# sehyun03/MulActSeg

Measured on AMD Instinct MI355X. Metric: superpixels scored/sec, higher is better.
Workload: dtype f32; 1 GPU; acquisition-round: PixBal+ban-ignore scorer on resident logits, Cityscapes pool shape [4,20,1024,2048] per step; per rank K single-pass scans (class prior + region sums + histograms) of its shard, then exchange 1 (all-gather class sums) + device class weights (k_class_weight) + weighted finalize + ban + exchange 2 (all-gather scores) + replicated K4 (keys, radix sort, fair-counting budget walk) ov; nseg=2048, id_dtype=int64, regions_scored=679936, budget_clicks=11159, regions_selected=6688

## Files before the change

include/mulactseg_hip.h:

```cpp
#ifndef MULACTSEG_HIP_H
#define MULACTSEG_HIP_H

#include <stddef.h>
#include <stdint.h>

#ifdef __cplusplus
extern "C" {
#endif

#define MAS_ID_I64 0
#define MAS_ID_I32 1
#define MAS_ID_U16 2
#define MAS_MAP_U8 3

#define MAS_MAX_CLASSES 32

#define MAS_SCORE_FRAC_BITS 40
#define MAS_PROB_FRAC_BITS 23
#define MAS_LOSS_FRAC_BITS 32

#define MAS_ABI_VERSION 9
int mas_abi_version(void);
const char* mas_error_string(int code);

// ... 54 lines not shown
#define MAS_GRAD_FRAC_BITS 44
int mas_fix_to_float(const int64_t* fix, int64_t n, int frac_bits, float* out, void* stream);

size_t mas_partial_loss_work_bytes(int N, int S, int C, int flags);
int mas_partial_loss_fwd_fused(const float* z, int h, int w, const void* spx, int spx_dtype, const uint8_t* mask, const uint8_t* targets,
                               int cols_stored, int cols_used, const uint32_t* bits, int N, int C, int H, int W, int S, float invT, int flags,
                               const float* weights, void* work, size_t work_bytes, float* losses, void* stream);
int mas_partial_loss_bwd_fused(const float* z, int h, int w, const void* spx, int spx_dtype, const uint8_t* mask, const uint32_t* bits,
                               const void* work, const float* grad, const float* weights, int N, int C, int H, int W, int S, float invT,
                               int flags, float* dz, int64_t* dzq_fix, void* stream);


int mas_region_keys(const float* score, const uint8_t* valid, const int32_t* img_rank, int64_t n_img, int S,
                    uint64_t* keys , void* stream);

size_t mas_select_workspace_bytes(int64_t n);

int mas_sort_keys_desc(const uint64_t* keys_in, int64_t n, uint64_t* keys_out, void* workspace, size_t ws_bytes,
                       void* stream);

int mas_budget_walk(const uint64_t* sorted_keys, int64_t n, const uint8_t* region_cost, const int32_t* img_of_rank,
                    int S, int64_t budget, int64_t max_out, int64_t* n_selected,
                    int32_t* sel_img, int32_t* sel_id, float* sel_score, void* workspace, size_t ws_bytes, void* stream);

int mas_region_reweight(float* score, const int32_t* dominant, int64_t n, int ban_class, const float* cls_w ,
                        void* stream);

int mas_dominant_hist(const int32_t* dominant, int64_t n, int C, uint64_t* counts , void* stream);

int mas_minmax_normalize(float* scores, int64_t n, uint32_t* scratch2, void* stream);


#define MAS_LABELS_BAD_VALUE 1

int mas_region_label_counts(const void* spx, int spx_dtype, const uint8_t* labels, int H, int W, int nseg, int num_classes, int trim_k,
                            int32_t* full , int32_t* trimmed , int32_t* status ,
                            void* stream);

int mas_region_multi_hot(const int32_t* full, const int32_t* trimmed, const uint8_t* listed, int nseg, int num_classes,
                         uint8_t* bits , int64_t* size , void* stream);

int mas_region_dominant(const int32_t* full, const uint8_t* listed, const int32_t* drawn , int nseg, int num_classes,
                        int generate_ignore, int32_t* choice , void* stream);

int mas_region_paint(const void* spx, int spx_dtype, const uint8_t* labels, int H, int W, int nseg, const int32_t* choice,
                     int generate_ignore, uint8_t* out , void* stream);
// ... 202 lines not shown
```

mulactseg_amd/_lib.py:

```python
import ctypes
import os

_HERE = os.path.dirname(os.path.abspath(__file__))
LIB_PATH = os.environ.get("MAS_LIB") or os.path.join(_HERE, "libmulactseg_hip.so")

ID_I64, ID_I32, ID_U16 = 0, 1, 2
MAP_U8 = 3
MAX_CLASSES = 32
LABELS_BAD_VALUE = 1
SCORE_FRAC, PROB_FRAC, LOSS_FRAC = 40, 23, 32
LOSS_CE, LOSS_GROUP, LOSS_GROUP_ONLY_MULTI, LOSS_DECOMP, LOSS_TCE = 1, 2, 4, 8, 16
ACC_WORDS = 8
GRAD_FRAC = 44
MS_MAX_SOURCES = 16

SK_DMA, SK_NOSPLIT = 1, 2
LOWRES_GENERIC = 1
STAGE2_THR_MEDIAN, STAGE2_THR_MIN = 0, 1
ABI_VERSION = 9

_c = ctypes
_vp, _i, _f, _i64, _d = _c.c_void_p, _c.c_int, _c.c_float, _c.c_int64, _c.c_double


class SkOpts(ctypes.Structure):
    _fields_ = [("flags", _c.c_uint), ("spin_limit", _c.c_uint), ("stamps", _c.c_void_p)]


SIGNATURES = {
    "mas_abi_version": (_i, []),
    "mas_error_string": (_c.c_char_p, [_i]),
    "mas_class_prob_sum": (_i, [_vp, _i, _i, _i, _i, _f, _vp, _vp]),
    "mas_bvsb_region_accum": (_i, [_vp, _vp, _i, _vp, _i, _i, _i, _i, _i, _f, _vp, _vp, _vp]),
    "mas_region_finalize": (_i, [_vp, _vp, _i64, _i, _i, _vp, _vp, _vp, _vp, _vp]),
    "mas_region_keys": (_i, [_vp, _vp, _vp, _i64, _i, _vp, _vp]),
    "mas_select_workspace_bytes": (_c.c_size_t, [_i64]),
    "mas_sort_keys_desc": (_i, [_vp, _i64, _vp, _vp, _c.c_size_t, _vp]),
    "mas_budget_walk": (_i, [_vp, _i64, _vp, _vp, _i, _i64, _i64, _vp, _vp, _vp, _vp, _vp, _c.c_size_t, _vp]),
    "mas_region_reweight": (_i, [_vp, _vp, _i64, _i, _vp, _vp]),
    "mas_dominant_hist": (_i, [_vp, _i64, _i, _vp, _vp]),
    "mas_minmax_normalize": (_i, [_vp, _i64, _vp, _vp]),
    "mas_region_label_counts": (_i, [_vp, _i, _vp, _i, _i, _i, _i, _i, _vp, _vp, _vp, _vp]),
    "mas_region_multi_hot": (_i, [_vp, _vp, _vp, _i, _i, _vp, _vp, _vp]),
    "mas_region_dominant": (_i, [_vp, _vp, _vp, _i, _i, _i, _vp, _vp]),
    "mas_region_paint": (_i, [_vp, _i, _vp, _i, _i, _i, _vp, _i, _vp, _vp]),
    "mas_spx_max_onehot": (_i, [_vp, _i, _vp, _i, _i, _i, _i, _i, _vp, _vp, _vp, _vp, _vp]),
    "mas_iou_counts": (_i, [_vp, _vp, _vp, _i64, _i, _i64, _vp, _vp]),
    "mas_logits_iou_counts": (_i, [_vp, _vp, _i, _i, _i, _i, _i, _i64, _vp, _vp]),
    "mas_lowres_iou_counts": (_i, [_vp, _vp, _i, _i, _i, _i, _i, _i, _i, _i64, _vp, _vp]),
    "mas_single_pass_accum": (_i, [_vp, _vp, _i, _i, _i, _i, _i, _i, _f, _vp, _vp, _vp, _vp]),
    "mas_single_pass_accum_lowres": (_i, [_vp, _i, _i, _vp, _i, _i, _i, _i, _i, _i, _f, _vp, _vp, _vp, _vp]),
    "mas_single_pass_accum_lowres_opt": (_i, [_vp, _i, _i, _vp, _i, _i, _i, _i, _i, _i, _f, _vp, _vp, _vp, _c.c_uint, _vp]),
    "mas_class_weight": (_i, [_vp, _i, _i, _i64, _i, _i, _d, _vp, _vp, _vp, _vp]),
    "mas_region_finalize_weighted": (_i, [_vp, _vp, _i64, _i, _vp, _i, _vp, _vp, _vp, _vp, _vp]),
    "mas_stage2_gather_protos": (_i, [_vp, _i, _i, _i, _i, _i, _vp, _i, _vp, _vp]),
    "mas_stage2_assign": (_i, [_vp, _i, _i, _i, _i, _i, _vp, _vp, _i, _vp, _vp, _vp, _vp, _vp]),
    "mas_stage2_adjacency": (_i, [_vp, _i, _i, _i, _vp, _vp, _vp]),
    "mas_stage2_propagate": (_i, [_vp, _i, _i, _i, _i, _i, _vp, _i, _vp, _vp, _vp, _vp, _vp, _vp, _vp, _vp]),
    "mas_stage2_thresholds_scratch_bytes": (_i64, [_i, _i]),
    "mas_stage2_thresholds": (_i, [_vp, _vp, _i, _i, _i, _vp, _i64, _vp, _vp]),
    "mas_aspp_dw3_fwd": (_i, [_vp, _vp, _vp, _vp, _i, _i, _i, _i, _i, _i, _i, _vp, _vp, _vp, _vp]),
# ... 135 lines not shown
```

mulactseg_amd/active_selection/engine.py:

```python
import numpy as np
import torch


class ShardPlan:

    def __init__(self, n_img, batch_size, rank=0, world=1):
        self.n_img, self.batch_size, self.rank, self.world = n_img, batch_size, rank, world
        self.n_batches = (n_img + batch_size - 1) // batch_size
        per = (self.n_batches + world - 1) // world
        self.batch_lo = min(rank * per, self.n_batches)
        self.batch_hi = min((rank + 1) * per, self.n_batches)
        self.img_lo = min(self.batch_lo * batch_size, n_img)
        self.img_hi = min(self.batch_hi * batch_size, n_img)
        self.per_rank_imgs = per * batch_size
        self.batch_of = (np.arange(n_img) // batch_size).astype(np.int32)

    @property
    def local_indices(self):
        return list(range(self.img_lo, self.img_hi))

    @property
    def n_local(self):
        return self.img_hi - self.img_lo

# ... 67 lines not shown

    def class_weight(self, prob_sum, hw, batch_size, n_batches, coeff):
        cum, w, w31 = self.ops.class_weight(prob_sum.contiguous(), hw, batch_size, n_batches, coeff)
        w._mas_w31 = w31
        return cum, w

    def finalize_weighted(self, class_sum, hist, cls_w, ban_class, want_hist_i64=False):
        w31 = None if cls_w is None else getattr(cls_w, '_mas_w31', None)
        if w31 is None:
            w = torch.ones(hist.shape[-1], dtype=torch.float32, device=hist.device) if cls_w is None else cls_w.detach().to(hist.device)
            w31 = (w.double() * 2147483648.0).floor().to(torch.int64).view(torch.int32)[::2].contiguous()
        return self.ops.region_finalize_weighted(class_sum, hist, w31, ban_class, want_hist_i64)

    def minmax_normalize_(self, scores):
        return self.ops.minmax_normalize_(scores)

    def region_reweight_(self, scores, dominant, ban_class, cls_w):
        return self.ops.region_reweight_(scores, dominant, ban_class, cls_w)

    def dominant_hist(self, dominant, C):
        return self.ops.dominant_hist(dominant, C)

    def select(self, scores, valid, img_rank, img_of_rank, region_cost, budget, max_out):
        keys = self.ops.region_keys(scores, valid, img_rank)
        skeys = self.ops.sort_keys_desc(keys)
        nsel, simg, sid, ssc = self.ops.budget_walk(skeys, region_cost, img_of_rank, scores.shape[1], budget, max_out)
        n = int(nsel.item())
        return n, simg[:n].cpu().numpy(), sid[:n].cpu().numpy(), ssc[:n].cpu().numpy()

    def local_head(self, plan, scores, valid, img_rank, max_out):
        lo, hi = plan.img_lo, plan.img_hi
        head = torch.zeros(max_out, dtype=torch.int64, device=scores.device)
        if hi > lo:
            keys = self.ops.region_keys(scores[lo:hi].contiguous(), None if valid is None else valid[lo:hi].contiguous(),
                                        img_rank[lo:hi].contiguous())
            m = min(keys.numel(), max_out)
            head[:m] = self.ops.sort_keys_desc(keys)[:m]
        return head

    def walk_heads(self, heads, region_cost, img_of_rank, S, budget, max_out):
        nsel, simg, sid, ssc = self.ops.budget_walk(self.ops.sort_keys_desc(heads), region_cost, img_of_rank, S, budget, max_out)
        n = int(nsel.item())
        return n, simg[:n].cpu().numpy(), sid[:n].cpu().numpy(), ssc[:n].cpu().numpy()

    def select_sharded(self, plan, scores, valid, img_rank, img_of_rank, region_cost, budget, max_out):
        head = self.local_head(plan, scores, valid, img_rank, max_out)
        merged = torch.empty(plan.world * max_out, dtype=torch.int64, device=scores.device)
        _dist().all_gather_into_tensor(merged, head)
        return self.walk_heads(merged, region_cost, img_of_rank, scores.shape[1], budget, max_out)


def default_backend(device):
    return HipBackend(device)


def select_regions(backend, plan, scores, valid, img_rank, img_of_rank, region_cost, budget, max_out):
    if plan.world > 1 and max_out is not None and _dist() is not None and hasattr(backend, 'select_sharded'):
        return backend.select_sharded(plan, scores, valid, img_rank, img_of_rank, region_cost, budget, max_out)
    return backend.select(scores, valid, img_rank, img_of_rank, region_cost, budget, max_out)


class AcquisitionRound:

    def __init__(self, n_img, n_channels, n_superpixels, batch_size, temperature, backend, rank=None, world=None,
                 single_pass=False):
        r, w = current_rank_world()
# ... 97 lines not shown
```

mulactseg_amd/csrc/select.hip:

```cpp
#include <cstring>

#include <rocprim/device/device_radix_sort.hpp>
#include <rocprim/device/device_scan.hpp>

#include "common.h"

namespace {

constexpr int kThreads = 256;

__device__ __forceinline__ unsigned order_bits(float f) {
    const unsigned b = mas_f2u(f);
    return (b & 0x80000000u) ? ~b : (b | 0x80000000u);
}
__device__ __forceinline__ float unorder_bits(unsigned o) {
    return mas_u2f((o & 0x80000000u) ? (o & 0x7fffffffu) : ~o);
}

inline int id_bits_for(int S) {
    int b = 1;
    while ((1LL << b) < S) ++b;
    return b;
}

// ... 100 lines not shown
        if (v != 0.0f) lo = o < lo ? o : lo;
        hi = o > hi ? o : hi;
    }
#pragma unroll
    for (int off = MAS_WAVE / 2; off > 0; off >>= 1) {
        const unsigned l2 = __shfl_down(lo, off, MAS_WAVE), h2 = __shfl_down(hi, off, MAS_WAVE);
        lo = l2 < lo ? l2 : lo;
        hi = h2 > hi ? h2 : hi;
    }
    if ((threadIdx.x & (MAS_WAVE - 1)) == 0) {
        atomicMin(&mm[0], lo);
        atomicMax(&mm[1], hi);
    }
}

__global__ void k_minmax_init(unsigned* mm) { mm[0] = 0xffffffffu; mm[1] = 0u; }

__global__ __launch_bounds__(kThreads) void k_minmax_apply(float* __restrict__ u, long long n, const unsigned* __restrict__ mm) {
    const long long i = (long long)blockIdx.x * kThreads + threadIdx.x;
    if (i >= n) return;
    const float mn = unorder_bits(mm[0]);
    const float mx = unorder_bits(mm[1]) - mn;
    u[i] = (u[i] - mn) / mx;
}

inline size_t align_up(size_t v) { return (v + 255) & ~(size_t)255; }

size_t sort_temp_bytes(long long n) {
    size_t bytes = 0;
    mas_u64* nul = nullptr;
    (void)rocprim::radix_sort_keys_desc(nullptr, bytes, nul, nul, (size_t)n, 0, 64, (hipStream_t)0);
    return bytes;
}
size_t scan_temp_bytes(long long n) {
    size_t bytes = 0;
    unsigned* nul = nullptr;
    (void)rocprim::inclusive_scan(nullptr, bytes, nul, nul, (size_t)n, rocprim::plus<unsigned>(), (hipStream_t)0);
    return bytes;
}

}

extern "C" size_t mas_select_workspace_bytes(int64_t n) {
    if (n <= 0) return 0;
    const size_t t = sort_temp_bytes(n), u = scan_temp_bytes(n);
    return align_up(t > u ? t : u) + 2 * align_up(sizeof(unsigned) * (size_t)n) + 256;
// ... 35 lines not shown
    hipStream_t st = static_cast<hipStream_t>(stream);
    const int b = id_bits_for(S);
    unsigned char* ws = static_cast<unsigned char*>(workspace);
    size_t temp = scan_temp_bytes(n);
    const size_t t = sort_temp_bytes(n);
    const size_t temp_region = align_up(t > temp ? t : temp);
    unsigned* cost = reinterpret_cast<unsigned*>(ws + temp_region);
    unsigned* prefix = reinterpret_cast<unsigned*>(ws + temp_region + align_up(sizeof(unsigned) * (size_t)n));
    const mas_u64* keys = reinterpret_cast<const mas_u64*>(sorted_keys);
    unsigned long long* nsel = reinterpret_cast<unsigned long long*>(n_selected);
    const long long nblk = (n + kThreads - 1) / kThreads;
    hipLaunchKernelGGL(k_set_u64, dim3(1), dim3(1), 0, st, nsel, (unsigned long long)n);
    hipLaunchKernelGGL(k_walk_cost, dim3((unsigned)nblk), dim3(kThreads), 0, st, keys, (long long)n, region_cost, img_of_rank, S, b, cost);
    hipError_t e = rocprim::inclusive_scan(ws, temp, cost, prefix, (size_t)n, rocprim::plus<unsigned>(), st);
    if (e != hipSuccess) return (int)e;
    hipLaunchKernelGGL(k_walk_find, dim3((unsigned)nblk), dim3(kThreads), 0, st, keys, prefix, (long long)n,
                       (unsigned long long)budget, nsel);
    const long long oblk = (max_out + kThreads - 1) / kThreads;
    hipLaunchKernelGGL(k_walk_emit, dim3((unsigned)oblk), dim3(kThreads), 0, st, keys, nsel, (long long)max_out, img_of_rank, b,
                       sel_img, sel_id, sel_score);
    return mas_launch_status();
}

extern "C" int mas_minmax_normalize(float* scores, int64_t n, uint32_t* scratch2, void* stream) {
    if (!scores || !scratch2) return MAS_ERR_NULL;
    if (n <= 0) return MAS_ERR_SHAPE;
    hipStream_t st = static_cast<hipStream_t>(stream);
    long long nblk = (n + kThreads - 1) / kThreads;
    hipLaunchKernelGGL(k_minmax_init, dim3(1), dim3(1), 0, st, scratch2);
    hipLaunchKernelGGL(k_minmax_nonzero, dim3((unsigned)(nblk > 1024 ? 1024 : nblk)), dim3(kThreads), 0, st, scores, (long long)n, scratch2);
    hipLaunchKernelGGL(k_minmax_apply, dim3((unsigned)nblk), dim3(kThreads), 0, st, scores, (long long)n, scratch2);
    return mas_launch_status();
}

extern "C" int mas_region_reweight(float* score, const int32_t* dominant, int64_t n, int ban_class, const float* cls_w, void* stream) {
    if (!score || !dominant) return MAS_ERR_NULL;
    if (n <= 0) return MAS_ERR_SHAPE;
    const long long nblk = (n + kThreads - 1) / kThreads;
    hipLaunchKernelGGL(k_region_reweight, dim3((unsigned)nblk), dim3(kThreads), 0, static_cast<hipStream_t>(stream), score, dominant,
                       (long long)n, ban_class, cls_w);
    return mas_launch_status();
}

extern "C" int mas_dominant_hist(const int32_t* dominant, int64_t n, int C, uint64_t* counts, void* stream) {
    if (!dominant || !counts) return MAS_ERR_NULL;
    if (n <= 0) return MAS_ERR_SHAPE;
// ... 8 lines not shown
```

mulactseg_amd/csrc/single_pass.hip:

```cpp
#include <cstdlib>
#include "common.h"

namespace {

constexpr int kThreads = 256;
constexpr int kTileW = 256;
constexpr int kTileH = 16;
constexpr int kLogSlots = 7;
constexpr int kSlots = 1 << kLogSlots;

__device__ __forceinline__ int table_slot(int* keys, int id) {
    unsigned h = ((unsigned)id * 2654435769u) >> (32 - kLogSlots);
    for (int probe = 0; probe < kSlots; ++probe) {
        int k = __hip_atomic_load(&keys[h], __ATOMIC_RELAXED, __HIP_MEMORY_SCOPE_WORKGROUP);
        if (k == id) return (int)h;
        if (k == -1) {
            int old = atomicCAS(&keys[h], -1, id);
            if (old == -1 || old == id) return (int)h;
        }
        h = (h + 1) & (kSlots - 1);
    }
    return -1;
}

// ... 481 lines not shown
                                                                        int C, const unsigned* __restrict__ w31, int ban_class,
                                                                        float* __restrict__ score, int* __restrict__ dominant,
                                                                        unsigned* __restrict__ count,
                                                                        long long* __restrict__ hist_i64) {
    extern __shared__ __attribute__((aligned(16))) unsigned char smem[];
    const int CP = C | 1;
    mas_u64* s_sum = reinterpret_cast<mas_u64*>(smem);
    unsigned* s_hist = reinterpret_cast<unsigned*>(s_sum + (size_t)kThreads * CP);
    const long long r0 = (long long)blockIdx.x * kThreads;
    const long long rows = (n_regions - r0) < kThreads ? (n_regions - r0) : kThreads;
    const long long words = rows * C;
    for (long long i = threadIdx.x; i < words; i += kThreads) {
        const int row = (int)(i / C), col = (int)(i - (long long)row * C);
        const unsigned hv = hist[r0 * C + i];
        s_sum[row * CP + col] = class_sum[r0 * C + i];
        s_hist[row * CP + col] = hv;
        if (hist_i64) hist_i64[r0 * C + i] = (long long)hv;
    }
    __syncthreads();
    if ((long long)threadIdx.x >= rows) return;
    const long long r = r0 + threadIdx.x;
    const unsigned* h = s_hist + threadIdx.x * CP;
    const mas_u64* cs = s_sum + threadIdx.x * CP;
    unsigned long long n = 0;
    unsigned best = 0;
    int arg = 0;
    uint64_t hi = 0, lo = 0;
    for (int c = 0; c < C; ++c) {
        const unsigned v = h[c];
        n += v;
        if (v > best) { best = v; arg = c; }
        if (v) mas_mac_u64_u32((uint64_t)cs[c], w31[c], &hi, &lo);
    }
    float sc = 0.0f;
    if (n) sc = mas_fixed_mean(mas_shr31_u128(hi, lo), n, MAS_SCORE_FRAC);
    if (ban_class >= 0 && arg == ban_class) sc = 0.0f;
    score[r] = sc;
    if (dominant) dominant[r] = arg;
    if (count) count[r] = (unsigned)n;
}

inline bool mas_ring_enabled() {
    static const bool on = [] { const char* e = getenv("MAS_SINGLE_PASS_RING"); return !(e && e[0] == '0'); }();
    return on;
}

// ... 122 lines not shown
    if (flags & ~MAS_LOWRES_GENERIC) return MAS_ERR_RANGE;
    hipStream_t st = static_cast<hipStream_t>(stream);
    mas_u64* ps = reinterpret_cast<mas_u64*>(prob_sum);
    mas_u64* cs = reinterpret_cast<mas_u64*>(class_sum);
    switch (C) {
        case 19: return dispatch_low_ids<19, true>(zq, h, w, spx, spx_dtype, B, C, H, W, S, invT, ps, cs, hist, flags, st);
        case 20: return dispatch_low_ids<20, true>(zq, h, w, spx, spx_dtype, B, C, H, W, S, invT, ps, cs, hist, flags, st);
        case 21: return dispatch_low_ids<21, true>(zq, h, w, spx, spx_dtype, B, C, H, W, S, invT, ps, cs, hist, flags, st);
        default: return MAS_ERR_CLASSES;
    }
}

extern "C" int mas_single_pass_accum_lowres(const float* zq, int h, int w, const void* spx, int spx_dtype, int B, int C, int H, int W, int S,
                                            float invT, uint64_t* prob_sum, uint64_t* class_sum, uint32_t* hist, void* stream) {
    return mas_single_pass_accum_lowres_opt(zq, h, w, spx, spx_dtype, B, C, H, W, S, invT, prob_sum, class_sum, hist, 0u, stream);
}

extern "C" int mas_region_finalize_weighted(const uint64_t* class_sum, const uint32_t* hist, int64_t n_regions, int C,
                                            const uint32_t* w31, int ban_class, float* score, int32_t* dominant, uint32_t* count,
                                            int64_t* hist_i64, void* stream) {
    if (!class_sum || !hist || !w31 || !score) return MAS_ERR_NULL;
    if (n_regions <= 0) return MAS_ERR_SHAPE;
    if (C < 1 || C > MAS_MAX_CLASSES) return MAS_ERR_CLASSES;
    const long long nblk = (n_regions + kThreads - 1) / kThreads;
    if (nblk > 0x7fffffffLL) return MAS_ERR_SHAPE;
    const size_t smem = (sizeof(mas_u64) + sizeof(unsigned)) * (size_t)kThreads * (C | 1);
    hipLaunchKernelGGL(k_region_finalize_weighted, dim3((unsigned)nblk), dim3(kThreads), smem, static_cast<hipStream_t>(stream),
                       reinterpret_cast<const mas_u64*>(class_sum), hist, (long long)n_regions, C, w31, ban_class, score, dominant,
                       count, reinterpret_cast<long long*>(hist_i64));
    return mas_launch_status();
}
```

mulactseg_amd/ops.py:

```python
import ctypes
import os

import numpy as np
import torch

from . import _lib

_ID_CODES = {torch.int64: _lib.ID_I64, torch.int32: _lib.ID_I32, torch.uint16: _lib.ID_U16,
             torch.int16: _lib.ID_U16}


def inv_temperature(T):
    return float(np.float32(1.0) / np.float32(T))


def _stream(t):
    return torch.cuda.current_stream(t.device).cuda_stream


def _need(t, name, dtype=None):
    if not t.is_cuda:
        raise _lib.MulActSegHipError("%s must live on the GPU (no CPU path exists)" % name)
    if dtype is not None and t.dtype != dtype:
        raise TypeError("%s must be %s, got %s" % (name, dtype, t.dtype))
# ... 282 lines not shown


def budget_walk(sorted_keys, region_cost, img_of_rank, S, budget, max_out=None):
    _need(sorted_keys, "sorted_keys", torch.int64)
    _need(img_of_rank, "img_of_rank", torch.int32)
    cost_bits = region_cost
    if cost_bits is not None:
        _need(cost_bits, "region_cost", torch.uint8)
    n = sorted_keys.numel()
    max_out = n if max_out is None else min(n, max_out)
    dev = sorted_keys.device
    lib = _lib.load()
    ws = torch.empty(lib.mas_select_workspace_bytes(n), dtype=torch.uint8, device=dev)
    nsel = torch.empty(1, dtype=torch.int64, device=dev)
    sel_img = torch.empty(max_out, dtype=torch.int32, device=dev)
    sel_id = torch.empty(max_out, dtype=torch.int32, device=dev)
    sel_score = torch.empty(max_out, dtype=torch.float32, device=dev)
    with torch.cuda.device(dev):
        _lib.check(lib.mas_budget_walk(sorted_keys.data_ptr(), n, cost_bits.data_ptr() if cost_bits is not None else None,
                                       img_of_rank.data_ptr(), S, int(budget), max_out, nsel.data_ptr(), sel_img.data_ptr(),
                                       sel_id.data_ptr(), sel_score.data_ptr(), ws.data_ptr(), ws.numel(), _stream(sorted_keys)),
                   "mas_budget_walk")
    return nsel, sel_img, sel_id, sel_score


def minmax_normalize_(scores):
    _need(scores, "scores", torch.float32)
    scratch = torch.empty(2, dtype=torch.int32, device=scores.device)
    with torch.cuda.device(scores.device):
        _lib.check(_lib.load().mas_minmax_normalize(scores.data_ptr(), scores.numel(), scratch.data_ptr(), _stream(scores)),
                   "mas_minmax_normalize")
    return scores


def iou_counts(outputs, outputs_all, targets, num_classes, ignore_label, counts=None):
    _need(targets, "targets", torch.int64)
    if outputs is not None:
        _need(outputs, "outputs", torch.int64)
    if outputs_all is not None:
        _need(outputs_all, "outputs_all", torch.int64)
    if counts is None:
        counts = torch.zeros(3 * num_classes + 3, dtype=torch.int64, device=targets.device)
    with torch.cuda.device(targets.device):
        _lib.check(_lib.load().mas_iou_counts(outputs.data_ptr() if outputs is not None else None,
                                              outputs_all.data_ptr() if outputs_all is not None else None,
                                              targets.data_ptr(), targets.numel(), num_classes, int(ignore_label),
# ... 1930 lines not shown
```

Before: 56.30 million superpixels/s.

## Replace full radix sort selection with histogram-threshold top-prefix select and fused sort-walk

Adds a prefix selection path. Two histogram passes over the score key bits find a threshold, a compaction pass keeps only the candidates above it (up to 8192), and one block runs a bitonic sort and the budget walk in shared memory, writing a single packed record. The aim is to avoid building and radix-sorting keys for all regions when only a few thousand can be selected. The record is read back in one pinned copy, and the path falls back to the full sort when candidates overflow the cap. The finalize kernel also gains a tiled variant, which adds complexity and possible tie and edge-case risks.

```diff
diff --git a/include/mulactseg_hip.h b/include/mulactseg_hip.h
--- a/include/mulactseg_hip.h
+++ b/include/mulactseg_hip.h
@@ -100,6 +100,12 @@
 int mas_budget_walk(const uint64_t* sorted_keys, int64_t n, const uint8_t* region_cost, const int32_t* img_of_rank,
                     int S, int64_t budget, int64_t max_out, int64_t* n_selected,
                     int32_t* sel_img, int32_t* sel_id, float* sel_score, void* workspace, size_t ws_bytes, void* stream);
+
+int64_t mas_select_prefix_cap(void);
+size_t mas_select_prefix_workspace_bytes(void);
+int mas_select_prefix(const float* score, const uint8_t* valid, const int32_t* img_rank, const int32_t* img_of_rank,
+                      const uint8_t* region_cost, int64_t n_img, int S, int64_t budget, int64_t max_out, int32_t* record,
+                      void* workspace, size_t ws_bytes, void* stream);
 
 int mas_region_reweight(float* score, const int32_t* dominant, int64_t n, int ban_class, const float* cls_w ,
                         void* stream);
diff --git a/mulactseg_amd/_lib.py b/mulactseg_amd/_lib.py
--- a/mulactseg_amd/_lib.py
+++ b/mulactseg_amd/_lib.py
@@ -37,6 +37,9 @@
     "mas_select_workspace_bytes": (_c.c_size_t, [_i64]),
     "mas_sort_keys_desc": (_i, [_vp, _i64, _vp, _vp, _c.c_size_t, _vp]),
     "mas_budget_walk": (_i, [_vp, _i64, _vp, _vp, _i, _i64, _i64, _vp, _vp, _vp, _vp, _vp, _c.c_size_t, _vp]),
+    "mas_select_prefix_cap": (_i64, []),
+    "mas_select_prefix_workspace_bytes": (_c.c_size_t, []),
+    "mas_select_prefix": (_i, [_vp, _vp, _vp, _vp, _vp, _i64, _i, _i64, _i64, _vp, _vp, _c.c_size_t, _vp]),
     "mas_region_reweight": (_i, [_vp, _vp, _i64, _i, _vp, _vp]),
     "mas_dominant_hist": (_i, [_vp, _i64, _i, _vp, _vp]),
     "mas_minmax_normalize": (_i, [_vp, _i64, _vp, _vp]),
diff --git a/mulactseg_amd/active_selection/engine.py b/mulactseg_amd/active_selection/engine.py
--- a/mulactseg_amd/active_selection/engine.py
+++ b/mulactseg_amd/active_selection/engine.py
@@ -113,11 +113,7 @@
         return self.ops.dominant_hist(dominant, C)
 
     def select(self, scores, valid, img_rank, img_of_rank, region_cost, budget, max_out):
-        keys = self.ops.region_keys(scores, valid, img_rank)
-        skeys = self.ops.sort_keys_desc(keys)
-        nsel, simg, sid, ssc = self.ops.budget_walk(skeys, region_cost, img_of_rank, scores.shape[1], budget, max_out)
-        n = int(nsel.item())
-        return n, simg[:n].cpu().numpy(), sid[:n].cpu().numpy(), ssc[:n].cpu().numpy()
+        return self.ops.select(scores, valid, img_rank, img_of_rank, region_cost, budget, max_out)
 
     def local_head(self, plan, scores, valid, img_rank, max_out):
         lo, hi = plan.img_lo, plan.img_hi
@@ -130,9 +126,7 @@
         return head
 
     def walk_heads(self, heads, region_cost, img_of_rank, S, budget, max_out):
-        nsel, simg, sid, ssc = self.ops.budget_walk(self.ops.sort_keys_desc(heads), region_cost, img_of_rank, S, budget, max_out)
-        n = int(nsel.item())
-        return n, simg[:n].cpu().numpy(), sid[:n].cpu().numpy(), ssc[:n].cpu().numpy()
+        return self.ops.walk_heads(heads, region_cost, img_of_rank, S, budget, max_out)
 
     def select_sharded(self, plan, scores, valid, img_rank, img_of_rank, region_cost, budget, max_out):
         head = self.local_head(plan, scores, valid, img_rank, max_out)
diff --git a/mulactseg_amd/csrc/select.hip b/mulactseg_amd/csrc/select.hip
--- a/mulactseg_amd/csrc/select.hip
+++ b/mulactseg_amd/csrc/select.hip
@@ -146,6 +146,267 @@
     const float mn = unorder_bits(mm[0]);
     const float mx = unorder_bits(mm[1]) - mn;
     u[i] = (u[i] - mn) / mx;
+}
+
+constexpr int kSelCap = 8192;
+constexpr int kSelBins = 4096;
+constexpr unsigned kNoBin = 0xffffffffu;
+constexpr int kSortThreads = 1024;
+constexpr int kSortItems = kSelCap / kSortThreads;
+constexpr int kHistItems = kSelBins / kThreads;
+enum { kStT1 = 0, kStAbove1, kStNeed2, kStM, kStCount, kStWords = 8 };
+constexpr size_t kSelStateBytes = 256;
+constexpr size_t kSelHistBytes = sizeof(unsigned) * kSelBins;
+constexpr size_t kSelZeroBytes = kSelStateBytes + 2 * kSelHistBytes;
+constexpr size_t kSelWorkspaceBytes = kSelZeroBytes + sizeof(mas_u64) * kSelCap;
+constexpr int kSortSlots = kSelCap + kSelCap / 8;
+constexpr size_t kSortSmemBytes = sizeof(mas_u64) * kSortSlots + sizeof(unsigned) * 32;
+
+__device__ __forceinline__ mas_u64 region_key(const float* __restrict__ score, const unsigned char* __restrict__ valid,
+                                              const int* __restrict__ img_rank, unsigned i, unsigned S, int id_bits) {
+    if (valid && !valid[i]) return 0;
+    const unsigned img = i / S;
+    const unsigned id = i - img * S;
+    const unsigned lo = ((unsigned)img_rank[img] << id_bits) | id;
+    return ((mas_u64)order_bits(score[i]) << 32) | lo;
+}
+
+__device__ void find_threshold(const unsigned* __restrict__ hist, unsigned need_cap, unsigned* s_scan, unsigned* out) {
+    const int tid = threadIdx.x;
+    unsigned h[kHistItems];
+    unsigned sum = 0;
+#pragma unroll
+    for (int e = 0; e < kHistItems; e += 4) {
+        const uint4 v = *reinterpret_cast<const uint4*>(hist + tid * kHistItems + e);
+        h[e] = v.x; h[e + 1] = v.y; h[e + 2] = v.z; h[e + 3] = v.w;
+        sum += v.x + v.y + v.z + v.w;
+    }
+    s_scan[tid] = sum;
+    if (tid == 0) { out[0] = kNoBin; out[1] = 0; }
+    __syncthreads();
+    for (int off = 1; off < kThreads; off <<= 1) {
+        const unsigned v = (tid + off < kThreads) ? s_scan[tid + off] : 0u;
+        __syncthreads();
+        s_scan[tid] += v;
+        __syncthreads();
+    }
+    const unsigned total = s_scan[0], incl = s_scan[tid], excl = incl - sum;
+    const unsigned need = need_cap < total ? need_cap : total;
+    if (need > 0 && excl < need && need <= incl) {
+        unsigned run = excl, T = kNoBin, above = 0;
+#pragma unroll
+        for (int e = kHistItems - 1; e >= 0; --e) {
+            if (T == kNoBin && run + h[e] >= need) { T = (unsigned)(tid * kHistItems + e); above = run; }
+            run += h[e];
+        }
+        out[0] = T;
+        out[1] = above;
+    }
+    if (tid == 0) out[2] = total;
+    __syncthreads();
+}
+
+template <int LEVEL>
+__global__ __launch_bounds__(kThreads) void k_prefix_hist(const float* __restrict__ score, const unsigned char* __restrict__ valid,
+                                                           const int* __restrict__ img_rank, unsigned n, unsigned S, int id_bits,
+                                                           unsigned max_out, unsigned* __restrict__ state,
+                                                           unsigned* __restrict__ hist1, unsigned* __restrict__ hist2) {
+    __shared__ unsigned s_h[kSelBins];
+    __shared__ unsigned s_scan[kThreads];
+    __shared__ unsigned s_out[4];
+    for (int b = threadIdx.x; b < kSelBins; b += kThreads) s_h[b] = 0;
+    unsigned T1 = 0;
+    if (LEVEL == 2) {
+        find_threshold(hist1, max_out, s_scan, s_out);
+        T1 = s_out[0];
+        if (blockIdx.x == 0 && threadIdx.x == 0) {
+            const unsigned need1 = max_out < s_out[2] ? max_out : s_out[2];
+            state[kStT1] = T1;
+            state[kStAbove1] = s_out[1];
+            state[kStNeed2] = need1 - s_out[1];
+        }
+        if (T1 == kNoBin) return;
+    }
+    __syncthreads();
+    for (unsigned long long i = (unsigned long long)blockIdx.x * kThreads + threadIdx.x; i < n; i += (unsigned long long)gridDim.x * kThreads) {
+        const mas_u64 k = region_key(score, valid, img_rank, (unsigned)i, S, id_bits);
+        if (LEVEL == 1) {
+            if (k) atomicAdd(&s_h[(unsigned)(k >> 52)], 1u);
+        } else {
+            if (k && (unsigned)(k >> 52) == T1) atomicAdd(&s_h[(unsigned)(k >> 40) & (kSelBins - 1)], 1u);
+        }
+    }
+    __syncthreads();
+    unsigned* hist = LEVEL == 1 ? hist1 : hist2;
+    for (int b = threadIdx.x; b < kSelBins; b += kThreads)
+        if (s_h[b]) atomicAdd(&hist[b], s_h[b]);
+}
+
+constexpr int kCompactItems = 4;
+
+__global__ __launch_bounds__(kThreads) void k_prefix_compact(const float* __restrict__ score, const unsigned char* __restrict__ valid,
+                                                              const int* __restrict__ img_rank, unsigned n, unsigned S, int id_bits,
+                                                              unsigned* __restrict__ state, const unsigned* __restrict__ hist2,
+                                                              mas_u64* __restrict__ cand) {
+    __shared__ unsigned s_scan[kThreads];
+    __shared__ unsigned s_out[4];
+    __shared__ unsigned s_wave[kThreads / MAS_WAVE + 1];
+    const unsigned T1 = state[kStT1];
+    if (T1 == kNoBin) return;
+    find_threshold(hist2, state[kStNeed2], s_scan, s_out);
+    const unsigned T2 = s_out[0];
+    if (T2 == kNoBin) return;
+    const unsigned m = state[kStAbove1] + s_out[1] + hist2[T2];
+    if (blockIdx.x == 0 && threadIdx.x == 0) state[kStM] = m;
+    if (m > (unsigned)kSelCap) return;
+    const unsigned cut = (T1 << 12) | T2;
+    const unsigned tid = threadIdx.x, lane = tid & (MAS_WAVE - 1), wave = tid / MAS_WAVE;
+    const unsigned long long i0 = (unsigned long long)blockIdx.x * (kThreads * kCompactItems) + tid;
+    mas_u64 k[kCompactItems];
+    unsigned cnt = 0;
+#pragma unroll
+    for (int e = 0; e < kCompactItems; ++e) {
+        const unsigned long long i = i0 + (unsigned)e * kThreads;
+        mas_u64 key = 0;
+        if (i < n) key = region_key(score, valid, img_rank, (unsigned)i, S, id_bits);
+        if (key == 0 || (unsigned)(key >> 40) < cut) key = 0;
+        k[e] = key;
+        cnt += key != 0;
+    }
+    unsigned incl = cnt;
+#pragma unroll
+    for (int off = 1; off < MAS_WAVE; off <<= 1) {
+        const unsigned up = __shfl_up(incl, off, MAS_WAVE);
+        if ((int)lane >= off) incl += up;
+    }
+    if (lane == MAS_WAVE - 1) s_wave[wave] = incl;
+    __syncthreads();
+    if (tid == 0) {
+        unsigned total = 0;
+#pragma unroll
+        for (int w = 0; w < kThreads / MAS_WAVE; ++w) { const unsigned c = s_wave[w]; s_wave[w] = total; total += c; }
+        s_wave[kThreads / MAS_WAVE] = total ? atomicAdd(&state[kStCount], total) : 0u;
+    }
+    __syncthreads();
+    unsigned at = s_wave[kThreads / MAS_WAVE] + s_wave[wave] + incl - cnt;
+#pragma unroll
+    for (int e = 0; e < kCompactItems; ++e) {
+        if (k[e]) {
+            if (at < (unsigned)kSelCap) cand[at] = k[e];
+            ++at;
+        }
+    }
+}
+
+__device__ __forceinline__ unsigned sort_slot(unsigned i) { return i + (i >> 3); }
+
+template <int STEPS>
+__device__ __forceinline__ void bitonic_group(mas_u64* s_key, unsigned P, unsigned k, unsigned j, unsigned tid) {
+    constexpr unsigned G = 1u << STEPS;
+    const unsigned jl = j >> (STEPS - 1);
+    for (unsigned g = tid; g < (P >> STEPS); g += kSortThreads) {
+        const unsigned base = ((g & ~(jl - 1)) << STEPS) | (g & (jl - 1));
+        const bool desc = (base & k) == 0;
+        mas_u64 v[G];
+#pragma unroll
+        for (unsigned a = 0; a < G; ++a) v[a] = s_key[sort_slot(base + a * jl)];
+#pragma unroll
+        for (int s = STEPS - 1; s >= 0; --s) {
+#pragma unroll
+            for (unsigned a = 0; a < G; ++a) {
+                if (a & (1u << s)) continue;
+                const unsigned b = a | (1u << s);
+                const mas_u64 x = v[a], y = v[b];
+                if (desc ? x < y : x > y) { v[a] = y; v[b] = x; }
+            }
+        }
+#pragma unroll
+        for (unsigned a = 0; a < G; ++a) s_key[sort_slot(base + a * jl)] = v[a];
+    }
+}
+
+__global__ __launch_bounds__(kSortThreads) void k_prefix_sort_walk(const mas_u64* __restrict__ cand, const unsigned* __restrict__ state,
+                                                                    const unsigned char* __restrict__ region_cost,
+                                                                    const int* __restrict__ img_of_rank, int S, int id_bits,
+                                                                    unsigned long long budget, int max_out, int* __restrict__ record) {
+    extern __shared__ __attribute__((aligned(16))) unsigned char s_raw[];
+    mas_u64* s_key = reinterpret_cast<mas_u64*>(s_raw);
+    unsigned* s_u = reinterpret_cast<unsigned*>(s_raw + sizeof(mas_u64) * kSortSlots);
+    const unsigned tid = threadIdx.x;
+    const unsigned m_raw = state[kStM];
+    const bool overflow = m_raw > (unsigned)kSelCap;
+    const unsigned m = overflow ? 0u : m_raw;
+    if (overflow) {
+        if (tid == 0) { record[0] = 0; record[1] = 0; record[2] = (int)m_raw; record[3] = 1; }
+        return;
+    }
+    unsigned P = 2;
+    while (P < m) P <<= 1;
+    for (unsigned i = tid; i < P; i += kSortThreads) s_key[sort_slot(i)] = i < m ? cand[i] : 0;
+    if (tid == 0) { s_u[16] = 0xffffffffu; s_u[17] = 0; }
+    __syncthreads();
+    for (unsigned k = 2; k <= P; k <<= 1) {
+        unsigned j = k >> 1;
+        while (j > 0) {
+            if (j >= 4) { bitonic_group<3>(s_key, P, k, j, tid); j >>= 3; }
+            else if (j == 2) { bitonic_group<2>(s_key, P, k, j, tid); j = 0; }
+            else { bitonic_group<1>(s_key, P, k, j, tid); j = 0; }
+            __syncthreads();
+        }
+    }
+    const unsigned base = tid * kSortItems;
+    const unsigned id_mask = (1u << id_bits) - 1u;
+    mas_u64 key[kSortItems];
+    int img[kSortItems];
+    unsigned c[kSortItems];
+#pragma unroll
+    for (int e = 0; e < kSortItems; ++e) key[e] = (base + e < P) ? s_key[sort_slot(base + e)] : 0;
+#pragma unroll
+    for (int e = 0; e < kSortItems; ++e) img[e] = img_of_rank[(unsigned)key[e] >> id_bits];
+#pragma unroll
+    for (int e = 0; e < kSortItems; ++e) c[e] = 1;
+    if (region_cost) {
+#pragma unroll
+        for (int e = 0; e < kSortItems; ++e) c[e] = (unsigned)region_cost[(long long)img[e] * S + (int)((unsigned)key[e] & id_mask)];
+    }
+    unsigned sum = 0, nv = 0;
+#pragma unroll
+    for (int e = 0; e < kSortItems; ++e) {
+        if (key[e]) { ++nv; sum += c[e]; }
+        c[e] = sum;
+    }
+    const unsigned lane = tid & (MAS_WAVE - 1), wave = tid / MAS_WAVE;
+    unsigned incl = sum;
+#pragma unroll
+    for (int off = 1; off < MAS_WAVE; off <<= 1) {
+        const unsigned up = __shfl_up(incl, off, MAS_WAVE);
+        if ((int)lane >= off) incl += up;
+    }
+    if (lane == MAS_WAVE - 1) s_u[wave] = incl;
+    __syncthreads();
+    unsigned before = incl - sum;
+    for (unsigned w = 0; w < wave; ++w) before += s_u[w];
+    unsigned first = 0xffffffffu;
+#pragma unroll
+    for (int e = kSortItems - 1; e >= 0; --e)
+        if (key[e] && (unsigned long long)(before + c[e]) > budget) first = base + e + 1;
+    if (first != 0xffffffffu) atomicMin(&s_u[16], first);
+    if (nv) atomicAdd(&s_u[17], nv);
+    __syncthreads();
+    const unsigned n_sel = s_u[16] < s_u[17] ? s_u[16] : s_u[17];
+    if (tid == 0) { record[0] = (int)n_sel; record[1] = 0; record[2] = (int)m_raw; record[3] = 0; }
+    int* sel_img = record + 4;
+    int* sel_id = sel_img + max_out;
+    float* sel_score = reinterpret_cast<float*>(sel_id + max_out);
+#pragma unroll
+    for (int e = 0; e < kSortItems; ++e) {
+        const unsigned i = base + e;
+        if (i >= (unsigned)max_out) break;
+        const bool taken = i < n_sel;
+        sel_img[i] = taken ? img[e] : -1;
+        sel_id[i] = taken ? (int)((unsigned)key[e] & id_mask) : -1;
+        sel_score[i] = taken ? unorder_bits((unsigned)(key[e] >> 32)) : 0.0f;
+    }
 }
 
 inline size_t align_up(size_t v) { return (v + 255) & ~(size_t)255; }
@@ -227,6 +488,54 @@
     return mas_launch_status();
 }
 
+extern "C" int64_t mas_select_prefix_cap(void) { return kSelCap; }
+
+extern "C" size_t mas_select_prefix_workspace_bytes(void) { return kSelWorkspaceBytes; }
+
+extern "C" int mas_select_prefix(const float* score, const uint8_t* valid, const int32_t* img_rank, const int32_t* img_of_rank,
+                                 const uint8_t* region_cost, int64_t n_img, int S, int64_t budget, int64_t max_out, int32_t* record,
+                                 void* workspace, size_t ws_bytes, void* stream) {
+    if (!score || !img_rank || !img_of_rank || !record || !workspace) return MAS_ERR_NULL;
+    if (n_img <= 0 || S <= 0 || max_out <= 0 || budget < 0) return MAS_ERR_SHAPE;
+    const int b = id_bits_for(S);
+    if (b > 24 || n_img > (1LL << (32 - b))) return MAS_ERR_RANGE;
+    const long long n = (long long)n_img * S;
+    if (n > 0x7fffffffLL || max_out > kSelCap) return MAS_ERR_RANGE;
+    if (ws_bytes < kSelWorkspaceBytes) return MAS_ERR_WORKSPACE;
+    if ((reinterpret_cast<uintptr_t>(workspace) & 15) || (reinterpret_cast<uintptr_t>(record) & 7)) return MAS_ERR_ALIGN;
+    hipStream_t st = static_cast<hipStream_t>(stream);
+    int dev = 0;
+    hipError_t e = hipGetDevice(&dev);
+    if (e != hipSuccess) return (int)e;
+    static bool attr_set[64] = {};
+    const bool cached = dev >= 0 && dev < 64;
+    if (!cached || !attr_set[dev]) {
+        e = hipFuncSetAttribute(reinterpret_cast<const void*>(&k_prefix_sort_walk), hipFuncAttributeMaxDynamicSharedMemorySize,
+                                (int)kSortSmemBytes);
+        if (e != hipSuccess) return (int)e;
+        if (cached) attr_set[dev] = true;
+    }
+    unsigned char* ws = static_cast<unsigned char*>(workspace);
+    unsigned* state = reinterpret_cast<unsigned*>(ws);
+    unsigned* hist1 = reinterpret_cast<unsigned*>(ws + kSelStateBytes);
+    unsigned* hist2 = reinterpret_cast<unsigned*>(ws + kSelStateBytes + kSelHistBytes);
+    mas_u64* cand = reinterpret_cast<mas_u64*>(ws + kSelZeroBytes);
+    e = hipMemsetAsync(ws, 0, kSelZeroBytes, st);
+    if (e != hipSuccess) return (int)e;
+    long long nblk = (n + (long long)kThreads * 8 - 1) / ((long long)kThreads * 8);
+    if (nblk > 2048) nblk = 2048;
+    const dim3 grid((unsigned)nblk), block(kThreads);
+    hipLaunchKernelGGL(k_prefix_hist<1>, grid, block, 0, st, score, valid, img_rank, (unsigned)n, (unsigned)S, b, (unsigned)max_out,
+                       state, hist1, hist2);
+    hipLaunchKernelGGL(k_prefix_hist<2>, grid, block, 0, st, score, valid, img_rank, (unsigned)n, (unsigned)S, b, (unsigned)max_out,
+                       state, hist1, hist2);
+    const dim3 cgrid((unsigned)((n + kThreads * kCompactItems - 1) / (kThreads * kCompactItems)));
+    hipLaunchKernelGGL(k_prefix_compact, cgrid, block, 0, st, score, valid, img_rank, (unsigned)n, (unsigned)S, b, state, hist2, cand);
+    hipLaunchKernelGGL(k_prefix_sort_walk, dim3(1), dim3(kSortThreads), kSortSmemBytes, st, cand, state, region_cost, img_of_rank, S, b,
+                       (unsigned long long)budget, (int)max_out, record);
+    return mas_launch_status();
+}
+
 extern "C" int mas_minmax_normalize(float* scores, int64_t n, uint32_t* scratch2, void* stream) {
     if (!scores || !scratch2) return MAS_ERR_NULL;
     if (n <= 0) return MAS_ERR_SHAPE;
diff --git a/mulactseg_amd/csrc/single_pass.hip b/mulactseg_amd/csrc/single_pass.hip
--- a/mulactseg_amd/csrc/single_pass.hip
+++ b/mulactseg_amd/csrc/single_pass.hip
@@ -527,6 +527,90 @@
     const long long r = r0 + threadIdx.x;
     const unsigned* h = s_hist + threadIdx.x * CP;
     const mas_u64* cs = s_sum + threadIdx.x * CP;
+    unsigned long long n = 0;
+    unsigned best = 0;
+    int arg = 0;
+    uint64_t hi = 0, lo = 0;
+    for (int c = 0; c < C; ++c) {
+        const unsigned v = h[c];
+        n += v;
+        if (v > best) { best = v; arg = c; }
+        if (v) mas_mac_u64_u32((uint64_t)cs[c], w31[c], &hi, &lo);
+    }
+    float sc = 0.0f;
+    if (n) sc = mas_fixed_mean(mas_shr31_u128(hi, lo), n, MAS_SCORE_FRAC);
+    if (ban_class >= 0 && arg == ban_class) sc = 0.0f;
+    score[r] = sc;
+    if (dominant) dominant[r] = arg;
+    if (count) count[r] = (unsigned)n;
+}
+
+constexpr int kFinRows = 64;
+constexpr int kFinSumLoads = kFinRows * MAS_MAX_CLASSES / 2 / kThreads;
+constexpr int kFinHistLoads = kFinRows * MAS_MAX_CLASSES / 4 / kThreads;
+static_assert(kFinSumLoads * kThreads * 2 == kFinRows * MAS_MAX_CLASSES && kFinHistLoads * kThreads * 4 == kFinRows * MAS_MAX_CLASSES,
+              "the per-thread load counts cover a tile of MAS_MAX_CLASSES columns exactly");
+
+__global__ __launch_bounds__(kThreads) void k_region_finalize_weighted_tile(const mas_u64* __restrict__ class_sum,
+                                                                             const unsigned* __restrict__ hist, int C,
+                                                                             const unsigned* __restrict__ w31, int ban_class,
+                                                                             float* __restrict__ score, int* __restrict__ dominant,
+                                                                             unsigned* __restrict__ count,
+                                                                             long long* __restrict__ hist_i64) {
+    extern __shared__ __attribute__((aligned(16))) unsigned char smem[];
+    const unsigned CP = (unsigned)C | 1u;
+    mas_u64* s_sum = reinterpret_cast<mas_u64*>(smem);
+    unsigned* s_hist = reinterpret_cast<unsigned*>(s_sum + (size_t)kFinRows * CP);
+    const unsigned tid = threadIdx.x;
+    const size_t w0 = (size_t)blockIdx.x * kFinRows * (size_t)C;
+    const ulonglong2* gsum = reinterpret_cast<const ulonglong2*>(class_sum + w0);
+    const uint4* ghist = reinterpret_cast<const uint4*>(hist + w0);
+    const unsigned nsum = (unsigned)(kFinRows * C) / 2, nhist = (unsigned)(kFinRows * C) / 4;
+    ulonglong2 sv[kFinSumLoads];
+    uint4 hv[kFinHistLoads];
+#pragma unroll
+    for (int k = 0; k < kFinSumLoads; ++k) {
+        const unsigned i = tid + k * kThreads;
+        sv[k] = i < nsum ? gsum[i] : ulonglong2{0, 0};
+    }
+#pragma unroll
+    for (int k = 0; k < kFinHistLoads; ++k) {
+        const unsigned i = tid + k * kThreads;
+        hv[k] = i < nhist ? ghist[i] : uint4{0, 0, 0, 0};
+    }
+#pragma unroll
+    for (int k = 0; k < kFinSumLoads; ++k) {
+        const unsigned i = tid + k * kThreads;
+        if (i < nsum) {
+            unsigned row = (2 * i) / (unsigned)C, col = 2 * i - row * (unsigned)C;
+            s_sum[row * CP + col] = sv[k].x;
+            if (++col == (unsigned)C) { col = 0; ++row; }
+            s_sum[row * CP + col] = sv[k].y;
+        }
+    }
+#pragma unroll
+    for (int k = 0; k < kFinHistLoads; ++k) {
+        const unsigned i = tid + k * kThreads;
+        if (i < nhist) {
+            const unsigned v[4] = {hv[k].x, hv[k].y, hv[k].z, hv[k].w};
+            unsigned row = (4 * i) / (unsigned)C, col = 4 * i - row * (unsigned)C;
+#pragma unroll
+            for (int e = 0; e < 4; ++e) {
+                s_hist[row * CP + col] = v[e];
+                if (++col == (unsigned)C) { col = 0; ++row; }
+            }
+            if (hist_i64) {
+                longlong2* o = reinterpret_cast<longlong2*>(hist_i64 + w0 + 4 * (size_t)i);
+                o[0] = longlong2{(long long)v[0], (long long)v[1]};
+                o[1] = longlong2{(long long)v[2], (long long)v[3]};
+            }
+        }
+    }
+    __syncthreads();
+    if (tid >= (unsigned)kFinRows) return;
+    const size_t r = (size_t)blockIdx.x * kFinRows + tid;
+    const unsigned* h = s_hist + tid * CP;
+    const mas_u64* cs = s_sum + tid * CP;
     unsigned long long n = 0;
     unsigned best = 0;
     int arg = 0;
@@ -695,11 +779,25 @@
     if (!class_sum || !hist || !w31 || !score) return MAS_ERR_NULL;
     if (n_regions <= 0) return MAS_ERR_SHAPE;
     if (C < 1 || C > MAS_MAX_CLASSES) return MAS_ERR_CLASSES;
-    const long long nblk = (n_regions + kThreads - 1) / kThreads;
-    if (nblk > 0x7fffffffLL) return MAS_ERR_SHAPE;
-    const size_t smem = (sizeof(mas_u64) + sizeof(unsigned)) * (size_t)kThreads * (C | 1);
-    hipLaunchKernelGGL(k_region_finalize_weighted, dim3((unsigned)nblk), dim3(kThreads), smem, static_cast<hipStream_t>(stream),
-                       reinterpret_cast<const mas_u64*>(class_sum), hist, (long long)n_regions, C, w31, ban_class, score, dominant,
-                       count, reinterpret_cast<long long*>(hist_i64));
+    hipStream_t st = static_cast<hipStream_t>(stream);
+    const mas_u64* cs = reinterpret_cast<const mas_u64*>(class_sum);
+    long long* h64 = reinterpret_cast<long long*>(hist_i64);
+    const bool aligned = (((uintptr_t)class_sum | (uintptr_t)hist | (uintptr_t)hist_i64) & 15) == 0;
+    const long long tiles = aligned ? n_regions / kFinRows : 0;
+    if (tiles > 0x7fffffffLL) return MAS_ERR_SHAPE;
+    if (tiles > 0) {
+        const size_t smem_tile = (sizeof(mas_u64) + sizeof(unsigned)) * (size_t)kFinRows * (C | 1);
+        hipLaunchKernelGGL(k_region_finalize_weighted_tile, dim3((unsigned)tiles), dim3(kThreads), smem_tile, st, cs, hist, C, w31,
+                           ban_class, score, dominant, count, h64);
+    }
+    const long long done = tiles * kFinRows, rest = n_regions - done;
+    if (rest > 0) {
+        const long long nblk = (rest + kThreads - 1) / kThreads;
+        if (nblk > 0x7fffffffLL) return MAS_ERR_SHAPE;
+        const size_t smem = (sizeof(mas_u64) + sizeof(unsigned)) * (size_t)kThreads * (C | 1);
+        hipLaunchKernelGGL(k_region_finalize_weighted, dim3((unsigned)nblk), dim3(kThreads), smem, st, cs + done * C, hist + done * C, rest,
+                           C, w31, ban_class, score + done, dominant ? dominant + done : nullptr, count ? count + done : nullptr,
+                           h64 ? h64 + done * C : nullptr);
+    }
     return mas_launch_status();
 }
diff --git a/mulactseg_amd/ops.py b/mulactseg_amd/ops.py
--- a/mulactseg_amd/ops.py
+++ b/mulactseg_amd/ops.py
@@ -328,6 +328,173 @@
                                        sel_id.data_ptr(), sel_score.data_ptr(), ws.data_ptr(), ws.numel(), _stream(sorted_keys)),
                    "mas_budget_walk")
     return nsel, sel_img, sel_id, sel_score
+
+
+RECORD_HEADER_WORDS = 4
+RECORD_OVERFLOW = 1
+_ONE_COPY_BYTES = 1 << 20
+_SELECT_WS, _SELECT_FULL_WS, _SELECT_WALK_WS, _SELECT_REC, _SELECT_HOST = {}, {}, {}, {}, {}
+SELECT_PATH_COUNTS = {"prefix": 0, "prefix_overflow": 0, "full": 0}
+last_select_path = None
+
+
+def _count_path(path):
+    global last_select_path
+    last_select_path = path
+    SELECT_PATH_COUNTS[path] += 1
+
+
+def select_prefix_cap():
+    return int(_lib.load().mas_select_prefix_cap())
+
+
+def select_prefix_eligible(n_img, S, max_out, cap=None):
+    if max_out is None:
+        return False
+    cap = select_prefix_cap() if cap is None else cap
+    return 1 <= min(int(max_out), n_img * S) <= cap and 0 < n_img * S < 2 ** 31
+
+
+def record_words(max_out):
+    return RECORD_HEADER_WORDS + 3 * int(max_out)
+
+
+def parse_record(words, max_out):
+    words = np.asarray(words, dtype=np.int32)
+    mo = int(max_out)
+    if words.ndim != 1 or words.size < record_words(mo):
+        raise ValueError("a record for max_out=%d has %d words, got %s" % (mo, record_words(mo), words.shape))
+    n = int(words[:2].view(np.int64)[0])
+    h = RECORD_HEADER_WORDS
+    return (n, int(words[2]), int(words[3]), words[h:h + mo], words[h + mo:h + 2 * mo],
+            words[h + 2 * mo:h + 3 * mo].view(np.float32))
+
+
+def _select_record(dev, max_out):
+    n = record_words(max_out)
+    rec = _stream_scratch(_SELECT_REC, dev, lambda: torch.empty(max(n, 1 << 14), dtype=torch.int32, device=dev), n)
+    return rec[:n]
+
+
+def _read_record(rec, max_out):
+    dev = rec.device
+    nw = rec.numel()
+    h = RECORD_HEADER_WORDS
+
+    def pinned(n):
+        return _stream_scratch(_SELECT_HOST, dev, lambda: torch.empty(max(n, 1 << 14), dtype=torch.int32).pin_memory(), n)
+
+    stream = torch.cuda.current_stream(dev)
+    if nw * 4 <= _ONE_COPY_BYTES:
+        host = pinned(nw)
+        host[:nw].copy_(rec, non_blocking=True)
+        stream.synchronize()
+        n, _, flags, img, rid, sc = parse_record(host[:nw].numpy(), max_out)
+        k = min(n, int(max_out))
+        return n, flags, img[:k].copy(), rid[:k].copy(), sc[:k].copy()
+    host = pinned(h)
+    host[:h].copy_(rec[:h], non_blocking=True)
+    stream.synchronize()
+    n, flags = int(host[:2].numpy().view(np.int64)[0]), int(host[3])
+    k = min(n, int(max_out))
+    host = pinned(h + 3 * k)
+    for j in range(3):
+        host[h + j * k:h + (j + 1) * k].copy_(rec[h + j * max_out:h + j * max_out + k], non_blocking=True)
+    stream.synchronize()
+    w = host[h:h + 3 * k].numpy()
+    return n, flags, w[:k].copy(), w[k:2 * k].copy(), w[2 * k:].view(np.float32).copy()
+
+
+def _select_inputs(scores, valid, img_rank, img_of_rank, region_cost):
+    _need(scores, "scores", torch.float32)
+    _need(img_rank, "img_rank", torch.int32)
+    _need(img_of_rank, "img_of_rank", torch.int32)
+    if scores.dim() != 2:
+        raise ValueError("scores must be [n_img, S]")
+    if valid is not None:
+        valid = _mask_u8(valid)
+        if tuple(valid.shape) != tuple(scores.shape):
+            raise ValueError("valid must be [n_img, S]")
+    if region_cost is not None:
+        _need(region_cost, "region_cost", torch.uint8)
+    return valid
+
+
+def select_prefix_record(scores, valid, img_rank, img_of_rank, region_cost, budget, max_out):
+    valid = _select_inputs(scores, valid, img_rank, img_of_rank, region_cost)
+    n_img, S = scores.shape
+    if not select_prefix_eligible(n_img, S, max_out):
+        raise ValueError("max_out=%s over %d x %d regions is outside the small-prefix path" % (max_out, n_img, S))
+    max_out = min(int(max_out), n_img * S)
+    dev = scores.device
+    lib = _lib.load()
+    nbytes = int(lib.mas_select_prefix_workspace_bytes())
+    ws = _stream_scratch(_SELECT_WS, dev, lambda: torch.empty(nbytes, dtype=torch.uint8, device=dev), nbytes)
+    rec = _select_record(dev, max_out)
+    with torch.cuda.device(dev):
+        _lib.check(lib.mas_select_prefix(scores.data_ptr(), _opt(valid), img_rank.data_ptr(), img_of_rank.data_ptr(), _opt(region_cost),
+                                         n_img, S, int(budget), max_out, rec.data_ptr(), ws.data_ptr(), ws.numel(), _stream(scores)),
+                   "mas_select_prefix")
+    return rec, max_out
+
+
+def sorted_walk_record(sorted_keys, region_cost, img_of_rank, S, budget, max_out, workspace=None):
+    _need(sorted_keys, "sorted_keys", torch.int64)
+    n = sorted_keys.numel()
+    max_out = n if max_out is None else min(n, int(max_out))
+    dev = sorted_keys.device
+    lib = _lib.load()
+    nbytes = int(lib.mas_select_workspace_bytes(max_out))
+    ws = workspace if workspace is not None and workspace.numel() >= nbytes else \
+        _stream_scratch(_SELECT_WALK_WS, dev, lambda: torch.empty(nbytes, dtype=torch.uint8, device=dev), nbytes)
+    rec = _select_record(dev, max_out)
+    h = RECORD_HEADER_WORDS
+    with torch.cuda.device(dev):
+        _lib.check(lib.mas_budget_walk(sorted_keys.data_ptr(), max_out, _opt(region_cost), img_of_rank.data_ptr(), S, int(budget), max_out,
+                                       rec.data_ptr(), rec[h:].data_ptr(), rec[h + max_out:].data_ptr(), rec[h + 2 * max_out:].data_ptr(),
+                                       ws.data_ptr(), ws.numel(), _stream(sorted_keys)), "mas_budget_walk")
+    return rec, max_out
+
+
+def select_full_record(scores, valid, img_rank, img_of_rank, region_cost, budget, max_out):
+    valid = _select_inputs(scores, valid, img_rank, img_of_rank, region_cost)
+    n_img, S = scores.shape
+    n = n_img * S
+    dev = scores.device
+    lib = _lib.load()
+    kb = (8 * n + 255) & ~255
+    nbytes = 2 * kb + int(lib.mas_select_workspace_bytes(n))
+    ws = _stream_scratch(_SELECT_FULL_WS, dev, lambda: torch.empty(nbytes, dtype=torch.uint8, device=dev), nbytes)
+    keys, skeys, temp = ws[:8 * n].view(torch.int64), ws[kb:kb + 8 * n].view(torch.int64), ws[2 * kb:]
+    with torch.cuda.device(dev):
+        _lib.check(lib.mas_region_keys(scores.data_ptr(), _opt(valid), img_rank.data_ptr(), n_img, S, keys.data_ptr(), _stream(scores)),
+                   "mas_region_keys")
+        _lib.check(lib.mas_sort_keys_desc(keys.data_ptr(), n, skeys.data_ptr(), temp.data_ptr(), temp.numel(), _stream(scores)),
+                   "mas_sort_keys_desc")
+    return sorted_walk_record(skeys, region_cost, img_of_rank, S, budget, max_out, workspace=temp)
+
+
+def select(scores, valid, img_rank, img_of_rank, region_cost, budget, max_out):
+    n_img, S = scores.shape
+    if select_prefix_eligible(n_img, S, max_out):
+        rec, mo = select_prefix_record(scores, valid, img_rank, img_of_rank, region_cost, budget, max_out)
+        n, flags, img, rid, sc = _read_record(rec, mo)
+        if not flags & RECORD_OVERFLOW:
+            _count_path("prefix")
+            return n, img, rid, sc
+        path = "prefix_overflow"
+    else:
+        path = "full"
+    rec, mo = select_full_record(scores, valid, img_rank, img_of_rank, region_cost, budget, max_out)
+    n, _, img, rid, sc = _read_record(rec, mo)
+    _count_path(path)
+    return n, img, rid, sc
+
+
+def walk_heads(heads, region_cost, img_of_rank, S, budget, max_out):
+    rec, mo = sorted_walk_record(sort_keys_desc(heads), region_cost, img_of_rank, S, budget, max_out)
+    n, _, img, rid, sc = _read_record(rec, mo)
+    return n, img, rid, sc
 
 
 def minmax_normalize_(scores):
```

Measured after the change: 56.69 million superpixels/s, median of 4. About the same (+0.7%).
